# ReplayCoding/mt-renderer

Hardware: AMD Instinct MI355X
Metric: Mtris/sec, 1M-tri 64-bone skinned scene @1920x1080 (higher is better)
Workload: dtype f32; 1 GPU; headline: 20 x mesh50k primitives = 1,000,000 strip triangles, 506,520 vertices x 24 B, 64-bone palette, debug-id shader, 1920x1080; triangles_per_frame=1000000, collective=none

## Files before the change

mt_renderer_amd/csrc/k_geom.hip:

```cpp
#include "geom_bins.h"
#include "geom_vertex.h"

#include <algorithm>
#include <type_traits>

namespace mtr {

struct PV {
    int32_t X, Y;
    float z, iw, up, vp;
    uint32_t flags;
};

enum { OC_XN = 1, OC_XP = 2, OC_YN = 4, OC_YP = 8, OC_ZN = 16, OC_ZP = 32 };

__device__ __forceinline__ uint32_t outcode(const VOut& c) {
    uint32_t oc = 0;
    if (c.x < -c.w) oc |= OC_XN;
    if (c.x > c.w) oc |= OC_XP;
    if (c.y < -c.w) oc |= OC_YN;
    if (c.y > c.w) oc |= OC_YP;
    if (c.z < 0.0f) oc |= OC_ZN;
    if (c.z > c.w) oc |= OC_ZP;
    return oc;
// ... 32 lines not shown
    if (cull == 0u ? A2 <= 0 : (A2 == 0 || (cull == 2u && A2 > 0))) return false;
    const bool flip = A2 < 0;
    const PV& b = flip ? c_in : b_in;
    const PV& c = flip ? b_in : c_in;
    int32_t xmin = min(a.X, min(b.X, c.X)), xmax = max(a.X, max(b.X, c.X));
    int32_t ymin = min(a.Y, min(b.Y, c.Y)), ymax = max(a.Y, max(b.Y, c.Y));
    int32_t px0 = (xmin + 127) >> 8, px1 = (xmax - 128) >> 8;
    int32_t py0 = (ymin + 127) >> 8, py1 = (ymax - 128) >> 8;
    px0 = max(px0, 0); py0 = max(py0, 0);
    px1 = min(px1, (int32_t)W - 1); py1 = min(py1, (int32_t)H - 1);
    if (px0 > px1 || py0 > py1) return false;
    if (small) *small = ((xmax - xmin) | (ymax - ymin)) < 512;
    r.h.bx0 = (uint16_t)(px0 >> MTR_BIN_SHIFT); r.h.bx1 = (uint16_t)(px1 >> MTR_BIN_SHIFT);
    r.h.by0 = (uint16_t)(py0 >> MTR_BIN_SHIFT); r.h.by1 = (uint16_t)(py1 >> MTR_BIN_SHIFT);
    r.a.X0 = a.X; r.a.Y0 = a.Y; r.a.X1 = b.X; r.a.Y1 = b.Y; r.a.X2 = c.X; r.a.Y2 = c.Y;
    r.a.z0 = a.z; r.a.z1 = b.z; r.a.z2 = c.z; r.a.mat = mat; r.a.pad0 = 0; r.a.pad1 = 0;
    r.b.iw0 = a.iw; r.b.iw1 = b.iw; r.b.iw2 = c.iw;
    r.b.up0 = a.up; r.b.up1 = b.up; r.b.up2 = c.up;
    r.b.vp0 = a.vp; r.b.vp1 = b.vp; r.b.vp2 = c.vp;
    r.b.pad0 = r.b.pad1 = r.b.pad2 = 0.0f;
    return true;
}

#ifndef MTR_SAMPLE_CULL
#define MTR_SAMPLE_CULL 1
#endif
#ifndef MTR_SAMPLE_FRAC
#define MTR_SAMPLE_FRAC 2u
#endif
__device__ __forceinline__ bool sample_cull(Rec& r, uint32_t W, uint32_t H) {
    const int32_t xmin = min(r.a.X0, min(r.a.X1, r.a.X2)), xmax = max(r.a.X0, max(r.a.X1, r.a.X2));
    const int32_t ymin = min(r.a.Y0, min(r.a.Y1, r.a.Y2)), ymax = max(r.a.Y0, max(r.a.Y1, r.a.Y2));
    const int32_t px0 = max((xmin + 127) >> 8, 0), py0 = max((ymin + 127) >> 8, 0);
    const bool two_x = min((xmax - 128) >> 8, (int32_t)W - 1) > px0, two_y = min((ymax - 128) >> 8, (int32_t)H - 1) > py0;
    const int32_t Sx = px0 * 256 + 128, Sy = py0 * 256 + 128;
    const int32_t u[3] = {Sx - r.a.X0, Sx - r.a.X1, Sx - r.a.X2}, v[3] = {Sy - r.a.Y0, Sy - r.a.Y1, Sy - r.a.Y2};
    int32_t e[3], ex[3], ey[3];
#pragma unroll
    for (int i = 0; i < 3; i++) {
        const int ia = (i + 1) % 3, ib = (i + 2) % 3;
        const int32_t ndx = u[ib] - u[ia], dy = v[ia] - v[ib];
        const int32_t bias = (((dy << 12) + ndx) - 1) >> 31;
        e[i] = __mul24(u[ib], v[ia]) - __mul24(u[ia], v[ib]) + bias;
        ex[i] = dy << 8; ey[i] = ndx << 8;
    }
    const bool m00 = (e[0] | e[1] | e[2]) >= 0;
    bool m10 = false, m01 = false, m11 = false;
    if (__ballot(two_x || two_y)) {
        m10 = two_x && ((e[0] + ex[0]) | (e[1] + ex[1]) | (e[2] + ex[2])) >= 0;
        m01 = two_y && ((e[0] + ey[0]) | (e[1] + ey[1]) | (e[2] + ey[2])) >= 0;
        m11 = two_x && two_y && ((e[0] + ex[0] + ey[0]) | (e[1] + ex[1] + ey[1]) | (e[2] + ex[2] + ey[2])) >= 0;
    }
    if (!(m00 || m10 || m01 || m11)) return false;
    if (two_x || two_y) {
        const int32_t qx0 = (m00 || m01) ? px0 : px0 + 1, qx1 = (m10 || m11) ? px0 + 1 : px0;
        const int32_t qy0 = (m00 || m10) ? py0 : py0 + 1, qy1 = (m01 || m11) ? py0 + 1 : py0;
        r.h.bx0 = (uint16_t)(qx0 >> MTR_BIN_SHIFT); r.h.bx1 = (uint16_t)(qx1 >> MTR_BIN_SHIFT);
        r.h.by0 = (uint16_t)(qy0 >> MTR_BIN_SHIFT); r.h.by1 = (uint16_t)(qy1 >> MTR_BIN_SHIFT);
    }
    return true;
}

#define MTR_MAX_POLY 8
__device__ __forceinline__ float guard_dist(const VOut& v, int plane) {
    return plane == 0 ? fmaf(64.0f, v.w, -v.x) : plane == 1 ? fmaf(64.0f, v.w, v.x) : plane == 2 ? fmaf(64.0f, v.w, -v.y) : fmaf(64.0f, v.w, v.y);
}
__device__ __forceinline__ VOut plane_lerp(const VOut& in, const VOut& out, float din, float dout) {
    const float t = din / (din - dout);
    VOut r;
    r.x = fmaf(t, out.x - in.x, in.x);
    r.y = fmaf(t, out.y - in.y, in.y);
    r.z = fmaf(t, out.z - in.z, in.z);
    r.w = fmaf(t, out.w - in.w, in.w);
    r.u = fmaf(t, out.u - in.u, in.u);
    r.v = fmaf(t, out.v - in.v, in.v);
    return r;
}
__device__ __forceinline__ VOut clip_lerp(const VOut& in, const VOut& out) {
    VOut r = plane_lerp(in, out, in.z, out.z);
    r.z = 0.0f;
    return r;
}

__device__ __forceinline__ void stage_palette(const GeomParams& P, uint32_t inst, float* s_pal, float* s_M) {
    if (threadIdx.x < 16) {
        float a = P.vp[threadIdx.x];
        if (P.model_mats) a = vp_model_elem(P.vp, P.model_mats, inst, threadIdx.x);
        s_M[threadIdx.x] = a;
    }
    if (P.palettes && P.npal) {
        const float4* src = reinterpret_cast<const float4*>(P.palettes + (size_t)inst * P.pal_stride);
        for (uint32_t i = threadIdx.x; i < P.npal * 4; i += blockDim.x) reinterpret_cast<float4*>(s_pal)[i] = src[i];
    }
    __syncthreads();
}

__device__ __forceinline__ uint32_t shading_position(const DPrim& pr, uint32_t lane) {
    return pr.topology == 4 ? (((lane & 31u) << 1) | (lane >> 5)) : lane;
}
__device__ __forceinline__ uint32_t fetch_index(const GeomParams& P, const DChunk& ch, const DPrim& pr, uint32_t lane) {
    const int32_t ps = (int32_t)ch.start - 2 + (int32_t)shading_position(pr, lane);
    return (ps >= 0 && (uint32_t)ps < pr.index_num) ? (uint32_t)P.ibuf[pr.index_ofs + (uint32_t)ps] : 0xFFFFu;
}

template <int MODE>
__device__ __forceinline__ void geom_chunk(const GeomParams& P, uint32_t inst, uint32_t c, const DChunk& ch, const DPrim& pr,
                                           bool skinned, const float* s_M, const float* s_pal, RecHdr* s_hdr, uint32_t* s_slot,
                                           float4* s_pv, uint32_t lane, uint32_t idx) {
    const uint32_t gid = P.chunk_base + inst * P.nchunks + c;
    const uint32_t mat = P.mat_base + inst * P.mat_inst_stride + ch.prim;
    const uint32_t W = P.fb.W, H = P.fb.H;
    const bool strip = pr.topology == 4;
    const DMat dmat = P.mats[mat];
    const bool want_b = pr.has_uv && dmat.shader == MTR_SH_TEXTURED;

    const uint32_t sp = shading_position(pr, lane);
    {
        const int32_t ps = (int32_t)ch.start - 2 + (int32_t)sp;
        const bool in_s = ps >= 0 && (uint32_t)ps < pr.index_num;
        const bool restart_s = !in_s || (strip && idx == 0xFFFFu);
        const uint32_t vid_s = idx + pr.index_base;
        const bool valid_s = !restart_s && vid_s < pr.vertex_num;
#ifndef MTR_ABL
#define MTR_ABL 0
#endif
#if MTR_ABL == 2
        VOut v; v.x = (float)(vid_s & 1023u) * 0.001f - 0.5f; v.y = (float)(vid_s >> 10) * 0.01f - 0.3f; v.z = 0.5f; v.w = 1.0f; v.u = v.v = 0.0f;
#else
        const VOut v = shade_vertex_mfma(P.vbuf, pr, vid_s, valid_s, s_M, s_pal, P.npal, MTR_ABL == 1 ? false : skinned, want_b);
#endif
        PV q;
        q.X = 0; q.Y = 0; q.z = 0.0f; q.iw = 0.0f; q.up = 0.0f; q.vp = 0.0f; q.flags = 0;
        if (valid_s) {
#if MTR_ABL == 6
            q.X = (int32_t)(v.x * 1000.0f); q.Y = (int32_t)(v.y * 1000.0f); q.z = v.z; q.flags = 2u;
#else
            q = project(v, W, H);
#endif
            q.flags |= 1u | (outcode(v) << 2);
        }
        const uint32_t fw = q.flags | (restart_s ? 0x100u : 0u) | (vid_s << 16);
        s_pv[sp] = make_float4(__int_as_float(q.X), __int_as_float(q.Y), q.z, __uint_as_float(fw));
        if (want_b) s_pv[64 + sp] = make_float4(q.iw, q.up, q.vp, 0.0f);
    }
    __builtin_amdgcn_fence(__ATOMIC_RELEASE, "wavefront");
    __builtin_amdgcn_wave_barrier();
    __builtin_amdgcn_fence(__ATOMIC_ACQUIRE, "wavefront");
    const int32_t p = (int32_t)ch.start - 2 + (int32_t)lane;
    const bool in_range = p >= 0 && (uint32_t)p < pr.index_num;
    PV me;
    me.iw = 0.0f; me.up = 0.0f; me.vp = 0.0f;
    uint32_t vid;
    bool is_restart;
    {
        const float4 a = s_pv[lane];
        const uint32_t fw = __float_as_uint(a.w);
        me.X = __float_as_int(a.x); me.Y = __float_as_int(a.y); me.z = a.z; me.flags = fw & 0xFFu;
        is_restart = (fw & 0x100u) != 0;
        vid = fw >> 16;
        if (want_b) {
            const float4 b = s_pv[64 + lane];
            me.iw = b.x; me.up = b.y; me.vp = b.z;
        }
    }

#if MTR_ABL == 3
    if (me.X == 0x7fffffff) P.fb.counters[CTR_OVERFLOW] = vid;
    return;
#endif
    const uint64_t R = __ballot(is_restart);
    const uint64_t below = R & ((1ull << lane) - 1ull);
    uint32_t q = 0;
    if (!is_restart) q = below ? lane - (63u - (uint32_t)__clzll((long long)below)) : ch.q_before + lane + 1u;
    bool tri, odd;
    if (strip) {
        tri = q >= 3 && lane >= 2;
        odd = ((q - 3) & 1) != 0;
    } else {
        tri = lane >= 2 && in_range && ((uint32_t)p % 3u == 2u);
        odd = false;
    }

    PV v1, v2;
    v1.iw = v1.up = v1.vp = v2.iw = v2.up = v2.vp = 0.0f;
#define MTR_SHR1(x) __builtin_amdgcn_update_dpp((int)(x), (int)(x), 0x138, 0xf, 0xf, false)
    v1.X = MTR_SHR1(me.X); v2.X = MTR_SHR1(v1.X);
    v1.Y = MTR_SHR1(me.Y); v2.Y = MTR_SHR1(v1.Y);
    v1.z = __int_as_float(MTR_SHR1(__float_as_int(me.z))); v2.z = __int_as_float(MTR_SHR1(__float_as_int(v1.z)));
    if (want_b) {
        v1.iw = __int_as_float(MTR_SHR1(__float_as_int(me.iw))); v2.iw = __int_as_float(MTR_SHR1(__float_as_int(v1.iw)));
        v1.up = __int_as_float(MTR_SHR1(__float_as_int(me.up))); v2.up = __int_as_float(MTR_SHR1(__float_as_int(v1.up)));
        v1.vp = __int_as_float(MTR_SHR1(__float_as_int(me.vp))); v2.vp = __int_as_float(MTR_SHR1(__float_as_int(v1.vp)));
    }
    v1.flags = (uint32_t)MTR_SHR1(me.flags); v2.flags = (uint32_t)MTR_SHR1(v1.flags);
    const uint32_t vid1 = (uint32_t)MTR_SHR1(vid), vid2 = (uint32_t)MTR_SHR1(vid1);
#undef MTR_SHR1

    const PV& ta = v2;
    const PV& tb = odd ? me : v1;
    const PV& tc = odd ? v1 : me;

    Rec r0, r1;
    uint32_t n_out = 0;
    bool empty = false;
    bool small = false;
    VOut poly[MTR_MAX_POLY];
    uint32_t n_poly = 0;
    const uint32_t f_and = ta.flags & tb.flags & tc.flags, f_or = ta.flags | tb.flags | tc.flags;
    tri = tri && (f_and & 1u);
    tri = tri && ((f_and >> 2) == 0);
#if MTR_ABL == 5
    tri = tri && ta.X == 0x7ffffff0;
#endif
    if (tri) {
        if (!((f_or >> 2) & OC_ZN) && (f_and & 2u)) {
            if (setup_tri(ta, tb, tc, W, H, mat, pr.cull, r0, &small)) n_out = 1;
        } else {
            const uint32_t ia = vid2, ib = odd ? vid : vid1, ic = odd ? vid1 : vid;
            float M[16];
#pragma unroll
            for (int i = 0; i < 16; i++) M[i] = s_M[i];
            VOut cv[3];
#pragma nounroll
            for (int i = 0; i < 3; i++) cv[i] = shade_vertex(P.vbuf, pr, i == 0 ? ia : (i == 1 ? ib : ic), M, s_pal, P.npal, skinned);
            int n = 3;
            if ((f_or >> 2) & OC_ZN) {
                n = 0;
#pragma unroll
                for (int i = 0; i < 3; i++) {
                    const VOut& pp = cv[i];
                    const VOut& qq = cv[(i + 1) % 3];
                    bool pin = !(pp.z < 0.0f), qin = !(qq.z < 0.0f);
                    if (pin) poly[n++] = pp;
                    if (pin != qin) poly[n++] = pin ? clip_lerp(pp, qq) : clip_lerp(qq, pp);
                }
            } else {
                poly[0] = cv[0]; poly[1] = cv[1]; poly[2] = cv[2];
            }
            if (n >= 3) {
                bool all_ok = true;
                for (int i = 0; i < n; i++) all_ok = all_ok && (project(poly[i], W, H).flags & 2u);
                if (all_ok) {
                    PV q0 = project(poly[0], W, H), q1 = project(poly[1], W, H), q2 = project(poly[2], W, H);
                    bool s0 = setup_tri(q0, q1, q2, W, H, mat, pr.cull, r0);
                    bool s1 = false;
                    if (n == 4) {
                        PV q3 = project(poly[3], W, H);
                        s1 = setup_tri(q0, q2, q3, W, H, mat, pr.cull, s0 ? r1 : r0);
                    }
                    n_out = (s0 ? 1u : 0u) + (s1 ? 1u : 0u);
                } else {
                    VOut tmp[MTR_MAX_POLY];
                    for (int plane = 0; plane < 4 && n >= 3; plane++) {
                        int m = 0;
                        for (int i = 0; i < n; i++) {
                            const VOut pp = poly[i], qq = poly[(i + 1) % n];
                            const float dp = guard_dist(pp, plane), dq = guard_dist(qq, plane);
                            const bool pin = !(dp < 0.0f), qin = !(dq < 0.0f);
                            if (pin && m < MTR_MAX_POLY) tmp[m++] = pp;
                            if (pin != qin && m < MTR_MAX_POLY) tmp[m++] = pin ? plane_lerp(pp, qq, dp, dq) : plane_lerp(qq, pp, dq, dp);
                        }
                        for (int i = 0; i < m; i++) poly[i] = tmp[i];
                        n = m;
                    }
                    if (n >= 3) n_poly = (uint32_t)n;
                }
            }
        }
    }

#if MTR_SAMPLE_CULL
    {
        const uint64_t sm = __ballot(small);
        if (sm && (uint32_t)__popcll(sm) * MTR_SAMPLE_FRAC >= (uint32_t)__popcll(__ballot(n_out != 0u)) && small && !sample_cull(r0, W, H)) {
            n_out = 0;
            empty = true;
        }
    }
#endif
    if (P.fb.own.world > 1 && empty) empty = rect_owned_any(P.fb.own, r0.h.bx0, r0.h.by0, r0.h.bx1, r0.h.by1, P.fb.nbx);
    if (P.fb.own.world > 1 && n_out) {
        const bool k0 = rect_owned_any(P.fb.own, r0.h.bx0, r0.h.by0, r0.h.bx1, r0.h.by1, P.fb.nbx);
        const bool k1 = n_out == 2 && rect_owned_any(P.fb.own, r1.h.bx0, r1.h.by0, r1.h.bx1, r1.h.by1, P.fb.nbx);
        if (!k0 && k1) r0 = r1;
        n_out = (k0 ? 1u : 0u) + (k1 ? 1u : 0u);
    }

    const uint32_t n_res = n_poly ? n_poly - 2u : n_out;
    uint32_t rank, total;
    const uint64_t b1 = __ballot(n_out >= 1), b2 = __ballot(n_out == 2);
    const uint32_t n_empty = (uint32_t)__popcll(__ballot(empty));
    if (!__ballot(n_poly != 0)) {
        const uint64_t lt = (1ull << lane) - 1ull;
        rank = (uint32_t)__popcll(b1 & lt) + (uint32_t)__popcll(b2 & lt);
        total = (uint32_t)__popcll(b1) + (uint32_t)__popcll(b2);
    } else {
        const uint32_t inc = wave_incl_scan_u32(n_res);
        rank = inc - n_res;
        total = (uint32_t)__builtin_amdgcn_readlane((int)inc, 63);
        if (total > MTR_CHUNK_SLOTS) {
            if (lane == 0) atomicOr(&P.fb.counters[CTR_OVERFLOW], 1u);
            total = 0;
        }
    }
    const uint32_t base = gid * MTR_CHUNK_SLOTS;
    if (lane == 0) {
        if (MODE == 0) {
            ChunkInfo ci = {base, total};
            P.fb.chunk_info[gid] = ci;
        }
        const uint32_t nrec = (uint32_t)__popcll(b1) + (uint32_t)__popcll(b2);
        const uint32_t nset = (total ? nrec : 0u) + n_empty;
        if (nset) atomicAdd(&P.fb.counters[MTR_CTR(CTR_REC, gid)], nset);
    }
    total = __builtin_amdgcn_readfirstlane(total);
    if (total == 0) return;
    const uint32_t solid = (dmat.shader != MTR_SH_TEXTURED && dmat.blend != MTR_DB_ADD && dmat.dstate == 3u) ? 1u : 0u;
    const uint32_t hard = (dmat.blend == MTR_DB_ADD || dmat.dstate != 3u) ? 1u : 0u;
    const uint32_t mflags = solid | ((dmat.blend != MTR_DB_OFF ? 1u : 0u) << 8) | (dmat.translucent << 16) | (hard << 17);
    r0.a.pad0 = dmat.rgba8; r0.a.pad1 = mflags;
    r1.a.pad0 = dmat.rgba8; r1.a.pad1 = mflags;
    auto put_rec = [&](uint32_t slot, const Rec& r) {
        const bool lg = rec_is_large(r.a);
        P.fb.rec_a[base + slot] = rec_pack(r.a, lg);
        if (lg) P.fb.rec_l[base + slot] = make_int4(r.a.X1, r.a.Y1, r.a.X2, r.a.Y2);
        if (MODE == 0) P.fb.rec_hdr[base + slot] = r.h;
        if (want_b) P.fb.rec_b[base + slot] = r.b;
        s_hdr[slot] = r.h;
    };
    if (n_out >= 1) put_rec(rank, r0);
    if (n_out == 2) put_rec(rank + 1, r1);
    if (n_poly) {
        uint32_t nvalid = 0;
        for (uint32_t k = 0; k + 2u < n_poly; k++) {
            Rec t;
            const PV q0 = project(poly[0], W, H), q1 = project(poly[k + 1], W, H), q2 = project(poly[k + 2], W, H);
            bool ok = setup_tri(q0, q1, q2, W, H, mat, pr.cull, t);
            if (ok && P.fb.own.world > 1) ok = rect_owned_any(P.fb.own, t.h.bx0, t.h.by0, t.h.bx1, t.h.by1, P.fb.nbx);
            if (ok) {
                t.a.pad0 = dmat.rgba8; t.a.pad1 = mflags;
                put_rec(rank + k, t);
                nvalid++;
            } else {
                const RecHdr hole = {1, 1, 0, 0};
                s_hdr[rank + k] = hole;
                if (MODE == 0) P.fb.rec_hdr[base + rank + k] = hole;
            }
        }
        if (nvalid) atomicAdd(&P.fb.counters[MTR_CTR(CTR_REC, gid + lane)], nvalid);
    }
    __builtin_amdgcn_fence(__ATOMIC_RELEASE, "wavefront");
    __builtin_amdgcn_wave_barrier();
    __builtin_amdgcn_fence(__ATOMIC_ACQUIRE, "wavefront");

#if MTR_ABL == 4
    return;
#endif
    for (uint32_t round = 0; round * 64 < total; ++round) {
        const uint32_t j = round * 64 + lane;
        bool act = j < total;
        RecHdr h = {0, 0, 0, 0};
        if (act) h = s_hdr[j];
        act = act && h.bx0 <= h.bx1;
        if (MODE == 2) {
            emit_bins_unordered(P.fb, h, act, gid, round, lane, s_slot);
        } else if (MODE == 1) {
            emit_bins<true>(P.fb, h, act, gid, round, lane);
        } else {
            count_bins(P.fb, h, act, lane);
        }
    }
}

#ifndef GEOM_OCC
#define GEOM_OCC 8
#define GEOM_OCC_SMALL 7
#endif
template <int MODE, bool CULL, int OCC>
__global__ __launch_bounds__(256, OCC) void k_geom(GeomParams P) {
    extern __shared__ __align__(16) float s_pal[];
    __shared__ RecHdr s_hdr[4][MTR_CHUNK_SLOTS + 4];
    __shared__ uint32_t s_slot[MODE == 2 ? 4 : 1][128];
    __shared__ float4 s_pv[4][128];
    __shared__ float s_M[16];
    const uint32_t lane = threadIdx.x & 63;
    const uint32_t wave = __builtin_amdgcn_readfirstlane(threadIdx.x >> 6);
    if (!CULL) {
        const uint32_t nblk = gridDim.x;
        const uint32_t per = (nblk + 7) / 8;
        const uint32_t blk = (blockIdx.x & 7) * per + (blockIdx.x >> 3);
        const uint32_t c = blk * 4 + wave;
        if (blk >= nblk) return;
        const bool has = c < P.nchunks;
        DChunk ch = {};
        DPrim pr = {};
        uint32_t idx = 0xFFFFu;
        if (has) { ch = P.chunks[c]; pr = P.prims[ch.prim]; idx = fetch_index(P, ch, pr, lane); }
        stage_palette(P, blockIdx.y, s_pal, s_M);
        if (!has) return;
        geom_chunk<MODE>(P, blockIdx.y, c, ch, pr, pr.skinnable && P.palettes && P.npal, s_M, s_pal, s_hdr[wave], s_slot[wave], s_pv[wave], lane, idx);
        return;
    }
    const uint32_t nxq = P.work_nx * 4u, ii = blockIdx.x / nxq, xq = blockIdx.x - ii * nxq, x = xq >> 2, q = xq & 3u;
    const uint32_t nlive = live_instances(P.inst_count, P.ninst);
    if (ii >= nlive) return;
    const size_t mi = (size_t)ii * P.work_nx + x;
    const uint32_t mword = reinterpret_cast<const uint32_t*>(P.work_mask)[mi >> 1];
    const uint32_t inst = P.inst_list ? P.inst_list[ii] : ii;
    const uint32_t m16 = (mi & 1u) ? mword >> 16 : mword & 0xFFFFu;
    const uint32_t k = (uint32_t)__popc(m16);
    if (q * 4u >= k) return;
    const uint32_t nth = q * 4u + wave;
    const bool has = nth < k;
    uint32_t mm = m16;
    for (uint32_t t = 0; t < nth && mm; t++) mm &= mm - 1u;
    const uint32_t c = x * 16u + (mm ? (uint32_t)__ffs((int)mm) - 1u : 0u);
    DChunk ch = {};
    DPrim pr = {};
    uint32_t idx = 0xFFFFu;
    if (has) { ch = P.chunks[c]; pr = P.prims[ch.prim]; idx = fetch_index(P, ch, pr, lane); }
    stage_palette(P, inst, s_pal, s_M);
    if (!has) return;
    geom_chunk<MODE>(P, inst, c, ch, pr, pr.skinnable && P.palettes && P.npal, s_M, s_pal, s_hdr[wave], s_slot[wave], s_pv[wave], lane, idx);
}

#define MTR_GEOM_REST_SPLIT 16u
template <int MODE>
__global__ __launch_bounds__(256) void k_geom_rest(GeomParams P) {
    extern __shared__ __align__(16) float s_pal[];
    __shared__ RecHdr s_hdr[4][MTR_CHUNK_SLOTS + 4];
    __shared__ uint32_t s_slot[MODE == 2 ? 4 : 1][128];
    __shared__ float4 s_pv[4][128];
    __shared__ float s_M[16];
    const uint32_t lane = threadIdx.x & 63;
    const uint32_t wave = __builtin_amdgcn_readfirstlane(threadIdx.x >> 6);
    const uint32_t split = min(P.work_nx, P.rest_split);
    const uint32_t ii = P.work_slot_base + blockIdx.x / split;
    const uint32_t nlive = live_instances(P.inst_count, P.ninst);
    if (ii >= nlive) return;
    const uint32_t inst = P.inst_list ? P.inst_list[ii] : ii;
    stage_palette(P, inst, s_pal, s_M);
    for (uint32_t x = blockIdx.x % split; x < P.work_nx; x += split) {
        const uint32_t m16 = P.work_mask[(size_t)ii * P.work_nx + x];
        const uint32_t k = (uint32_t)__popc(m16);
        for (uint32_t nth = wave; nth < k; nth += 4) {
            uint32_t mm = m16;
            for (uint32_t t = 0; t < nth; t++) mm &= mm - 1u;
            const uint32_t c = x * 16u + (uint32_t)__ffs((int)mm) - 1u;
            const DChunk ch = P.chunks[c];
            const DPrim pr = P.prims[ch.prim];
            geom_chunk<MODE>(P, inst, c, ch, pr, pr.skinnable && P.palettes && P.npal, s_M, s_pal, s_hdr[wave], s_slot[wave], s_pv[wave], lane,
                             fetch_index(P, ch, pr, lane));
        }
    }
}
__global__ __launch_bounds__(256) void k_vertex_stage(GeomParams P, uint32_t prim, float* out_clip, float* out_uv) {
    extern __shared__ __align__(16) float s_pal[];
    __shared__ float s_M[16];
    stage_palette(P, 0, s_pal, s_M);
    const DPrim pr = P.prims[prim];
    const bool skinned = pr.skinnable && P.palettes && P.npal;
    const uint32_t v = blockIdx.x * blockDim.x + threadIdx.x;
    if ((v & ~63u) >= pr.vertex_num) return;
    const VOut o = shade_vertex_mfma(P.vbuf, pr, v, v < pr.vertex_num, s_M, s_pal, P.npal, skinned, true);
    if (v >= pr.vertex_num) return;
    out_clip[4 * v + 0] = o.x; out_clip[4 * v + 1] = o.y; out_clip[4 * v + 2] = o.z; out_clip[4 * v + 3] = o.w;
    out_uv[2 * v + 0] = o.u; out_uv[2 * v + 1] = o.v;
}

}

template <class F>
static void with_geom_mode(const FrameBuffers& fb, F launch) {
    if (fb.direct && fb.unordered) launch(std::integral_constant<int, 2>());
    else if (fb.direct) launch(std::integral_constant<int, 1>());
    else launch(std::integral_constant<int, 0>());
}
template <bool CULL>
static void launch_geom(const GeomParams& p, dim3 grid, size_t lds, hipStream_t s) {
    with_geom_mode(p.fb, [&](auto mode) {
        constexpr int MODE = decltype(mode)::value;
        if (p.small_draw) hipLaunchKernelGGL((mtr::k_geom<MODE, CULL, GEOM_OCC_SMALL>), grid, dim3(256), lds, s, p);
        else hipLaunchKernelGGL((mtr::k_geom<MODE, CULL, GEOM_OCC>), grid, dim3(256), lds, s, p);
    });
}
void mtr_launch_geom(const GeomParams& p, hipStream_t s) {
    if (p.nchunks == 0 || p.ninst == 0) return;
    size_t lds = (size_t)p.npal * 64;
    if (p.work_mask) {
        uint32_t slots = p.ninst;
        if (p.inst_count && p.fb.own.world > 1) slots = std::min<uint32_t>(p.ninst, (2u * p.ninst + p.fb.own.world - 1) / p.fb.own.world + 64u);
        if (p.inst_count && (p.slots_hint & 0x80000000u)) {
            const uint32_t h = p.slots_hint & 0x7FFFFFFFu;
            slots = std::min<uint32_t>(p.ninst, h + h / 8u + 4u);
        }
        if ((uint64_t)(p.ninst - slots) * p.work_nx * 4u <= 20000u) slots = p.ninst;
        if (p.slots_override) slots = std::min<uint32_t>(p.ninst, p.slots_override);
        dim3 grid(p.work_nx * 4u * slots);
        launch_geom<true>(p, grid, lds, s);
        if (slots < p.ninst) {
            GeomParams r = p;
            r.work_slot_base = slots;
            r.rest_split = (p.inst_count && (p.slots_hint & 0x80000000u) && !p.slots_override) ? MTR_GEOM_REST_SPLIT / 4u : MTR_GEOM_REST_SPLIT;
            dim3 rest((p.ninst - slots) * std::min<uint32_t>(p.work_nx, r.rest_split));
            with_geom_mode(p.fb, [&](auto mode) { hipLaunchKernelGGL((mtr::k_geom_rest<decltype(mode)::value>), rest, dim3(256), lds, s, r); });
        }
        return;
    }
    uint32_t nblk = (p.nchunks + 3) / 4;
    nblk = (nblk + 7) / 8 * 8;
    dim3 grid(nblk, p.ninst);
    launch_geom<false>(p, grid, lds, s);
}

void mtr_launch_vertex_stage(const GeomParams& p, uint32_t prim, float* out_clip, float* out_uv, hipStream_t s) {
    hipLaunchKernelGGL(mtr::k_vertex_stage, dim3(256), dim3(256), (size_t)p.npal * 64, s, p, prim, out_clip, out_uv);
}
```

mt_renderer_amd/csrc/mtr_internal.h:

```cpp
#pragma once
#include <hip/hip_runtime.h>
#include <stdint.h>

#define MTR_BIN 16
#define MTR_BIN_SHIFT 4
#define MTR_SUB 8
#define MTR_CHUNK_NEW 62
#define MTR_CHUNK_SLOTS 124
#define MTR_GUARD_BAND 1048576.0f

enum { MTR_SH_DEBUG = 0, MTR_SH_TEXTURED = 1, MTR_SH_CONST = 2 };

struct DPrim {
    uint32_t vertex_base, vertex_num, stride;
    uint32_t index_ofs, index_num, index_base;
    uint32_t topology;
    uint32_t pos_fmt, pos_cnt, pos_off;
    uint32_t uv_fmt, uv_cnt, uv_off, has_uv;
    uint32_t joint_off, weight_off, skinnable;
    uint32_t aligned4;
    uint32_t parts_no;
    uint32_t cull;
};

struct DChunk {
    uint32_t prim;
    uint32_t start;
    uint32_t q_before;
    uint32_t ntris;
    uint32_t b_first;
    uint32_t b_count;
    uint32_t b_flags;
    uint32_t pad;
};

struct BoneBox {
    float cx, cy, cz;
    float ex, ey, ez;
    uint32_t joint;
    uint32_t pad;
};
#define MTR_BOX_UNSKINNED 0xFFFFFFFFu
#define MTR_CULL_CTR_WORDS 32
#define MTR_CHUNK_MAX_BOXES 15

struct CompMat {
    float C[12];
    float A[12];
};

struct DMat {
    uint32_t shader;
    uint32_t rgba8;
    uint32_t blend;
    uint32_t tw, th;
    uint32_t translucent;
    const uint8_t* tex;
    uint32_t tlevels;
    uint32_t dstate;
};
enum { MTR_TR_RGBA8 = 0, MTR_TR_BC1 = 1, MTR_TR_BC7 = 2 };
enum { MTR_DB_OFF = 0, MTR_DB_ALPHA = 1, MTR_DB_ADD = 2 };

struct RecHdr {
    uint16_t bx0, by0, bx1, by1;
};
struct RecA {
    int32_t X0, Y0, X1, Y1;
    int32_t X2, Y2;
    float z0, z1;
    float z2;
    uint32_t mat;
    uint32_t pad0, pad1;
};
struct RecP {
    uint4 q0, q1;
};
#define MTR_REC_LARGE_SENTINEL 0x8000u
#define MTR_MAX_TEXTURED_MATERIALS (1u << 24)

__device__ __forceinline__ bool rec_is_large(const RecA& a) {
    const int32_t d1x = a.X1 - a.X0, d1y = a.Y1 - a.Y0, d2x = a.X2 - a.X0, d2y = a.Y2 - a.Y0;
    return d1x < -32767 || d1x > 32767 || d1y < -32767 || d1y > 32767 || d2x < -32767 || d2x > 32767 || d2y < -32767 || d2y > 32767;
}
// ... 93 lines not shown

template <int CTRL, class T>
__device__ __forceinline__ T dpp_mov(T v) {
    return __builtin_bit_cast(T, __builtin_amdgcn_update_dpp(0, __builtin_bit_cast(int, v), CTRL, 0xf, 0xf, false));
}
template <class T, class Op>
__device__ __forceinline__ T row_reduce(T v, Op op) {
    v = op(v, dpp_mov<0x128>(v));
    v = op(v, dpp_mov<0x124>(v));
    v = op(v, dpp_mov<0x122>(v));
    v = op(v, dpp_mov<0x121>(v));
    return v;
}
template <class T, class Op>
__device__ __forceinline__ T wave_reduce(T v, Op op) {
    v = row_reduce(v, op);
    const int i = __builtin_bit_cast(int, v);
    const T r0 = __builtin_bit_cast(T, __builtin_amdgcn_readlane(i, 0)), r1 = __builtin_bit_cast(T, __builtin_amdgcn_readlane(i, 16));
    const T r2 = __builtin_bit_cast(T, __builtin_amdgcn_readlane(i, 32)), r3 = __builtin_bit_cast(T, __builtin_amdgcn_readlane(i, 48));
    return op(op(r0, r1), op(r2, r3));
}

__device__ __forceinline__ float vp_model_elem(const float (&vp)[16], const float* model_mats, uint32_t inst, uint32_t e) {
    __builtin_assume(e < 16);
    const uint32_t i = e & 3u, c = e >> 2;
    const float* B = model_mats + (size_t)inst * 16;
    float a = 0.0f;
#pragma unroll
    for (int k = 0; k < 4; k++) a = fmaf(vp[k * 4 + i], B[c * 4 + k], a);
    return a;
}

__device__ __forceinline__ uint32_t live_instances(const uint32_t* count, uint32_t ninst) {
    asm("" : "+s"(ninst));
    if (count) ninst = *count;
    return ninst;
}
#endif

enum { CTR_ENTRIES = 1, CTR_SEGS = 2, CTR_OVERFLOW = 3, CTR_SHARD_BASE = 32, CTR_SHARD_STRIDE = 32, CTR_NSHARDS = 128,
       CTR_REC = 0, CTR_ENT = 1, CTR_SEG = 2, CTR_CULL = 3 ,
       CTR_NUM = CTR_SHARD_BASE + CTR_NSHARDS * CTR_SHARD_STRIDE };
#define MTR_CTR(kind, k) (CTR_SHARD_BASE + ((k) & (CTR_NSHARDS - 1)) * CTR_SHARD_STRIDE + (kind))

struct FrameBuffers {
    RecHdr* rec_hdr;
    RecP* rec_a;
    int4* rec_l;
    RecB* rec_b;
    ChunkInfo* chunk_info;
    unsigned long long* bin_count;
    unsigned long long* bin_fill;
    uint32_t* bin_start;
    uint32_t* seg_start;
    uint32_t* entries;
    Seg* segs;
    uint32_t* counters;
    uint32_t rec_cap, entry_cap, seg_cap;
    uint32_t W, H, nbx, nby;
    Ownership own;
    uint32_t direct, qcap, scap;
    uint32_t unordered;
};

__device__ __forceinline__ void bin_queue_done(const FrameBuffers& fb, uint32_t bin) {
    if (fb.direct) {
        fb.bin_count[bin] = fb.bin_fill[bin];
        fb.bin_fill[bin] = 0ull;
    }
}

__device__ __forceinline__ void bin_queue(const FrameBuffers& fb, uint32_t bin, uint32_t& ent_lo, uint32_t& n_ent,
                                          uint32_t& seg_lo, uint32_t& n_seg) {
    if (fb.direct) {
        const unsigned long long f = fb.bin_fill[bin];
        ent_lo = bin * fb.qcap; seg_lo = bin * fb.scap;
        n_ent = min((uint32_t)f, fb.qcap); n_seg = min((uint32_t)(f >> 32), fb.scap);
    } else {
        ent_lo = fb.bin_start[bin]; n_ent = fb.bin_start[bin + 1] - ent_lo;
        seg_lo = fb.seg_start[bin]; n_seg = fb.seg_start[bin + 1] - seg_lo;
    }
}

struct GeomParams {
    const uint8_t* vbuf;
    const uint16_t* ibuf;
    const DPrim* prims;
    const DChunk* chunks;
    const BoneBox* boxes;
    uint32_t nchunks;
    uint32_t ninst;
    const uint16_t* work_mask;
    uint32_t work_nx;
    uint32_t work_slot_base;
    uint32_t rest_split;
    uint32_t slots_override;
    uint32_t small_draw;
    const uint32_t* inst_list;
    const uint32_t* inst_count;
    uint32_t slots_hint;
    const float* model_mats;
    const float* palettes;
    uint32_t npal, pal_stride;
    float vp[16];
    uint32_t chunk_base;
    uint32_t mat_base, mat_inst_stride;
    const DMat* mats;
    FrameBuffers fb;
};

struct alignas(64) TileHead {
    uint32_t grid;
    uint32_t own_count;
    uint32_t nbx, nbins;
    uint32_t W, H;
    uint32_t direct, qcap, scap;
    uint32_t xcd_run;
    uint32_t nbx_mul, nbx_shift, run_mul, run_shift;
    uint32_t zero_nwords, nhint;
    const uint32_t* own_list;
    uint32_t* entries;
    unsigned long long* bin_fill;
    uint32_t* bin_start;
    uint32_t* seg_start;
    uint32_t* counters;
    RecP* rec_a;
    uint32_t* zero_next;
    uint32_t* zero_words;
    uint32_t* host_status;
};
static_assert(sizeof(TileHead) == 192 && alignof(TileHead) == 64, "TileHead is three 64-byte lines");

struct TileParams {
    TileHead head;
    FrameBuffers fb;
    const DMat* mats;
    uint8_t* color;
    float* depth;
    uint32_t clear_rgba8;
    float clear_depth;
    uint8_t* bin_flag;
    uint32_t mixed;
    uint32_t* zero_next;
    uint32_t* host_status;
    uint32_t vis_waves;
    uint32_t xcd_run;
    uint32_t* zero_words;
    uint32_t zero_nwords;
    uint32_t* hint_out;
    uint32_t nhint;
    uint16_t hint_word[4], hint_slot[4];
};
#define MTR_TILE_PARAMS 1

static inline uint32_t mtr_vis_waves_for(uint32_t forced, uint32_t own_count) {
    if (forced) return forced;
    return own_count <= 1536 ? 8u : own_count <= 4096 ? 4u : 2u;
}

void mtr_launch_geom(const GeomParams& p, hipStream_t s);
void mtr_launch_scan(const FrameBuffers& fb, hipStream_t s);
void mtr_launch_fill(const FrameBuffers& fb, uint32_t total_chunks, hipStream_t s);
void mtr_launch_tile(const TileParams& p, bool textured, hipStream_t s);
void mtr_launch_tile_vis(const TileParams& p, bool textured, hipStream_t s);
void mtr_launch_alpha_min(const uint8_t* rgba, size_t npixels, uint32_t* out_min, hipStream_t s);
void mtr_launch_vertex_stage(const GeomParams& p, uint32_t prim, float* out_clip, float* out_uv, hipStream_t s);
void mtr_launch_bc1_decode(const uint8_t* blocks, uint8_t* rgba, uint32_t w, uint32_t h, hipStream_t s);
void mtr_launch_bc7_decode(const uint8_t* blocks, uint8_t* rgba, uint32_t w, uint32_t h, hipStream_t s);
void mtr_launch_pack_shard(const uint8_t* color, uint8_t* dst, uint32_t W, uint32_t H, const uint32_t* own_list, uint32_t own_count,
                           uint32_t stride_bins, hipStream_t s);
void mtr_launch_unpack_shards(const uint8_t* gathered, uint8_t* color, uint32_t W, uint32_t H, const uint32_t* src_of_bin, hipStream_t s);
struct CullParams {
    const BoneBox* boxes;
    uint32_t nboxes;
    uint32_t ninst;
    const float* model_mats;
    const float* palettes;
    uint32_t npal, pal_stride;
    float vp[16];
    uint32_t W, H, nbx, nby;
    Ownership own;
    uint32_t* list;
    uint32_t* count;
    CompMat* comp;
    uint32_t ncomp;
    uint16_t* work_mask;
    uint32_t* strad;
    uint32_t nchunks;
    uint32_t* counters;
};
void mtr_launch_cull_instances(const CullParams& p, hipStream_t s);
struct ChunkCullParams {
// ... 163 lines not shown
```

Before: 23430 Mtris/s.

## Pack hot geometry kernel args into cache-line head and overlap palette loads

Adds a 256-byte, 64-byte-aligned GeomHead at the start of the kernel arguments holding the hot scalars, pointers and VP matrix, read through scalar loads. Cold framebuffer fields are reloaded late from the kernarg segment. Palette staging is split into an issue phase and a finish phase so the palette global loads overlap the chunk, prim and material fetches. Material rows can also be prefetched alongside prims for the small-occupancy variant. This aims to cut kernel-prologue latency and scalar-load stalls, at the cost of a larger kernarg block and fragile inline-asm scheduling hints.

```diff
diff --git a/mt_renderer_amd/csrc/k_geom.hip b/mt_renderer_amd/csrc/k_geom.hip
--- a/mt_renderer_amd/csrc/k_geom.hip
+++ b/mt_renderer_amd/csrc/k_geom.hip
@@ -138,36 +138,128 @@
     return r;
 }
 
-__device__ __forceinline__ void stage_palette(const GeomParams& P, uint32_t inst, float* s_pal, float* s_M) {
-    if (threadIdx.x < 16) {
-        float a = P.vp[threadIdx.x];
-        if (P.model_mats) a = vp_model_elem(P.vp, P.model_mats, inst, threadIdx.x);
+#define MTR_GEOM_BLOCK 256u
+struct PalStage {
+    float4 v0;
+    float a[4], b[4];
+    const float4* src;
+    uint32_t n4;
+    bool composed;
+};
+__device__ __forceinline__ PalStage palette_issue(const GeomParams& P, const GeomHead& h, uint32_t inst, float* s_M) {
+    PalStage st;
+    st.v0 = make_float4(0.0f, 0.0f, 0.0f, 0.0f);
+#pragma unroll
+    for (int k = 0; k < 4; k++) st.a[k] = st.b[k] = 0.0f;
+    st.n4 = h.palettes ? h.npal * 4 : 0u;
+    st.src = reinterpret_cast<const float4*>(h.palettes + (size_t)inst * h.pal_stride);
+    st.composed = h.model_mats != nullptr;
+    if (threadIdx.x < st.n4) st.v0 = st.src[threadIdx.x];
+    if (st.composed) {
+        if (threadIdx.x < 16) {
+            const uint32_t i = threadIdx.x & 3u, c = threadIdx.x >> 2;
+            const float* B = h.model_mats + (size_t)inst * 16;
+#pragma unroll
+            for (int k = 0; k < 4; k++) { st.a[k] = P.vp[k * 4 + i]; st.b[k] = B[c * 4 + k]; }
+        }
+    } else if (threadIdx.x == 0) {
+#pragma unroll
+        for (int c = 0; c < 4; c++) reinterpret_cast<float4*>(s_M)[c] = make_float4(h.vp[c * 4], h.vp[c * 4 + 1], h.vp[c * 4 + 2], h.vp[c * 4 + 3]);
+    }
+    return st;
+}
+__device__ __forceinline__ void palette_finish(const PalStage& st, float* s_pal, float* s_M) {
+    if (st.composed && threadIdx.x < 16) {
+        float a = 0.0f;
+        PalStage t = st;
+        asm volatile("" : "+v"(t.a[0]), "+v"(t.a[1]), "+v"(t.a[2]), "+v"(t.a[3]), "+v"(t.b[0]), "+v"(t.b[1]), "+v"(t.b[2]), "+v"(t.b[3]));
+#pragma unroll
+        for (int k = 0; k < 4; k++) a = fmaf(t.a[k], t.b[k], a);
         s_M[threadIdx.x] = a;
     }
-    if (P.palettes && P.npal) {
-        const float4* src = reinterpret_cast<const float4*>(P.palettes + (size_t)inst * P.pal_stride);
-        for (uint32_t i = threadIdx.x; i < P.npal * 4; i += blockDim.x) reinterpret_cast<float4*>(s_pal)[i] = src[i];
-    }
+    if (threadIdx.x < st.n4) reinterpret_cast<float4*>(s_pal)[threadIdx.x] = st.v0;
+    for (uint32_t i = threadIdx.x + MTR_GEOM_BLOCK; i < st.n4; i += MTR_GEOM_BLOCK) reinterpret_cast<float4*>(s_pal)[i] = st.src[i];
     __syncthreads();
+}
+__device__ __forceinline__ void stage_palette(const GeomParams& P, const GeomHead& h, uint32_t inst, float* s_pal, float* s_M) {
+    const PalStage st = palette_issue(P, h, inst, s_M);
+    palette_finish(st, s_pal, s_M);
+}
+
+template <bool CULL>
+__device__ __forceinline__ GeomHead geom_head(const GeomParams& P) {
+    const GeomHead h = P.head;
+    asm volatile("" ::"s"(h.grid), "s"(h.nchunks), "s"(h.chunk_base), "s"(h.mat_base), "s"(h.mat_inst_stride), "s"(h.npal), "s"(h.pal_stride),
+                 "s"(h.chunks), "s"(h.prims), "s"(h.ibuf), "s"(h.vbuf), "s"(h.mats), "s"(h.palettes), "s"(h.model_mats), "s"(h.W), "s"(h.H),
+                 "s"(h.world));
+    asm volatile("" ::"s"(h.vp[0]), "s"(h.vp[1]), "s"(h.vp[2]), "s"(h.vp[3]), "s"(h.vp[4]), "s"(h.vp[5]), "s"(h.vp[6]), "s"(h.vp[7]), "s"(h.vp[8]),
+                 "s"(h.vp[9]), "s"(h.vp[10]), "s"(h.vp[11]), "s"(h.vp[12]), "s"(h.vp[13]), "s"(h.vp[14]), "s"(h.vp[15]));
+    if (CULL) asm volatile("" ::"s"(h.ninst), "s"(h.work_nx), "s"(h.work_mask), "s"(h.inst_list), "s"(h.inst_count));
+    return h;
+}
+typedef const __attribute__((address_space(4))) uint32_t* ConstWords;
+template <class T>
+__device__ __forceinline__ T load_words(ConstWords q) {
+    static_assert(sizeof(T) % 4 == 0 && alignof(T) >= 4, "whole dwords");
+    struct Words { uint32_t w[sizeof(T) / 4]; } r;
+#pragma unroll
+    for (uint32_t i = 0; i < sizeof(T) / 4; i++) r.w[i] = q[i];
+    return __builtin_bit_cast(T, r);
+}
+template <class T>
+__device__ __forceinline__ T load_const(const T* p) {
+    return load_words<T>((ConstWords)p);
+}
+
+__device__ __forceinline__ FrameBuffers geom_late(const GeomHead& h) {
+    typedef const GeomParams __attribute__((address_space(4)))* GeomArgs;
+    GeomArgs q = (GeomArgs)__builtin_amdgcn_kernarg_segment_ptr();
+    asm volatile("" : "+s"(q));
+    FrameBuffers fb = load_words<FrameBuffers>((ConstWords)&q->fb);
+    fb.rec_a = q->head.rec_a; fb.rec_l = q->head.rec_l; fb.rec_b = q->head.rec_b;
+    fb.entries = q->head.entries; fb.bin_fill = q->head.bin_fill; fb.counters = q->head.counters;
+    fb.nbx = q->head.nbx; fb.qcap = q->head.qcap;
+    asm volatile("" ::"s"(fb.rec_a), "s"(fb.rec_l), "s"(fb.rec_b), "s"(fb.entries), "s"(fb.bin_fill), "s"(fb.counters), "s"(fb.nbx), "s"(fb.qcap));
+    fb.W = h.W; fb.H = h.H;
+    fb.own.world = h.world;
+    return fb;
+}
+
+__device__ __forceinline__ uint32_t geom_live_instances(const GeomHead& h) {
+    uint32_t n = h.ninst;
+    asm("" : "+s"(n));
+    if (h.inst_count) n = load_const(h.inst_count);
+    return n;
 }
 
 __device__ __forceinline__ uint32_t shading_position(const DPrim& pr, uint32_t lane) {
     return pr.topology == 4 ? (((lane & 31u) << 1) | (lane >> 5)) : lane;
 }
-__device__ __forceinline__ uint32_t fetch_index(const GeomParams& P, const DChunk& ch, const DPrim& pr, uint32_t lane) {
+__device__ __forceinline__ uint32_t fetch_index(const GeomHead& h, const DChunk& ch, const DPrim& pr, uint32_t lane) {
     const int32_t ps = (int32_t)ch.start - 2 + (int32_t)shading_position(pr, lane);
-    return (ps >= 0 && (uint32_t)ps < pr.index_num) ? (uint32_t)P.ibuf[pr.index_ofs + (uint32_t)ps] : 0xFFFFu;
-}
-
-template <int MODE>
-__device__ __forceinline__ void geom_chunk(const GeomParams& P, uint32_t inst, uint32_t c, const DChunk& ch, const DPrim& pr,
-                                           bool skinned, const float* s_M, const float* s_pal, RecHdr* s_hdr, uint32_t* s_slot,
+    return (ps >= 0 && (uint32_t)ps < pr.index_num) ? (uint32_t)h.ibuf[pr.index_ofs + (uint32_t)ps] : 0xFFFFu;
+}
+template <bool ROW>
+__device__ __forceinline__ void fetch_prim_mat(const GeomHead& h, uint32_t inst, const DChunk& ch, DPrim& pr, DMat& dm) {
+    pr = load_const(h.prims + ch.prim);
+    if (ROW) {
+        dm = load_const(h.mats + (h.mat_base + inst * h.mat_inst_stride + ch.prim));
+        asm volatile("" ::"s"(pr.index_ofs), "s"(dm.shader), "s"(dm.rgba8), "s"(dm.blend), "s"(dm.translucent), "s"(dm.dstate));
+    } else {
+        asm volatile("" ::"s"(pr.index_ofs));
+    }
+    __builtin_amdgcn_sched_barrier(0);
+}
+
+template <int MODE, bool ROW>
+__device__ __forceinline__ void geom_chunk(const GeomHead& P, uint32_t inst, uint32_t c, const DChunk& ch,
+                                           const DPrim& pr, const DMat& row, bool skinned, const float* s_M, const float* s_pal, RecHdr* s_hdr, uint32_t* s_slot,
                                            float4* s_pv, uint32_t lane, uint32_t idx) {
     const uint32_t gid = P.chunk_base + inst * P.nchunks + c;
     const uint32_t mat = P.mat_base + inst * P.mat_inst_stride + ch.prim;
-    const uint32_t W = P.fb.W, H = P.fb.H;
+    const uint32_t W = P.W, H = P.H;
     const bool strip = pr.topology == 4;
-    const DMat dmat = P.mats[mat];
+    const DMat dmat = ROW ? row : load_const(P.mats + mat);
     const bool want_b = pr.has_uv && dmat.shader == MTR_SH_TEXTURED;
 
     const uint32_t sp = shading_position(pr, lane);
@@ -221,7 +313,7 @@
     }
 
 #if MTR_ABL == 3
-    if (me.X == 0x7fffffff) P.fb.counters[CTR_OVERFLOW] = vid;
+    if (me.X == 0x7fffffff) P.counters[CTR_OVERFLOW] = vid;
     return;
 #endif
     const uint64_t R = __ballot(is_restart);
@@ -325,6 +417,7 @@
         }
     }
 
+    const FrameBuffers fb = geom_late(P);
 #if MTR_SAMPLE_CULL
     {
         const uint64_t sm = __ballot(small);
@@ -334,10 +427,10 @@
         }
     }
 #endif
-    if (P.fb.own.world > 1 && empty) empty = rect_owned_any(P.fb.own, r0.h.bx0, r0.h.by0, r0.h.bx1, r0.h.by1, P.fb.nbx);
-    if (P.fb.own.world > 1 && n_out) {
-        const bool k0 = rect_owned_any(P.fb.own, r0.h.bx0, r0.h.by0, r0.h.bx1, r0.h.by1, P.fb.nbx);
-        const bool k1 = n_out == 2 && rect_owned_any(P.fb.own, r1.h.bx0, r1.h.by0, r1.h.bx1, r1.h.by1, P.fb.nbx);
+    if (P.world > 1 && empty) empty = rect_owned_any(fb.own, r0.h.bx0, r0.h.by0, r0.h.bx1, r0.h.by1, fb.nbx);
+    if (P.world > 1 && n_out) {
+        const bool k0 = rect_owned_any(fb.own, r0.h.bx0, r0.h.by0, r0.h.bx1, r0.h.by1, fb.nbx);
+        const bool k1 = n_out == 2 && rect_owned_any(fb.own, r1.h.bx0, r1.h.by0, r1.h.bx1, r1.h.by1, fb.nbx);
         if (!k0 && k1) r0 = r1;
         n_out = (k0 ? 1u : 0u) + (k1 ? 1u : 0u);
     }
@@ -355,7 +448,7 @@
         rank = inc - n_res;
         total = (uint32_t)__builtin_amdgcn_readlane((int)inc, 63);
         if (total > MTR_CHUNK_SLOTS) {
-            if (lane == 0) atomicOr(&P.fb.counters[CTR_OVERFLOW], 1u);
+            if (lane == 0) atomicOr(&fb.counters[CTR_OVERFLOW], 1u);
             total = 0;
         }
     }
@@ -363,11 +456,11 @@
     if (lane == 0) {
         if (MODE == 0) {
             ChunkInfo ci = {base, total};
-            P.fb.chunk_info[gid] = ci;
+            fb.chunk_info[gid] = ci;
         }
         const uint32_t nrec = (uint32_t)__popcll(b1) + (uint32_t)__popcll(b2);
         const uint32_t nset = (total ? nrec : 0u) + n_empty;
-        if (nset) atomicAdd(&P.fb.counters[MTR_CTR(CTR_REC, gid)], nset);
+        if (nset) atomicAdd(&fb.counters[MTR_CTR(CTR_REC, gid)], nset);
     }
     total = __builtin_amdgcn_readfirstlane(total);
     if (total == 0) return;
@@ -378,10 +471,10 @@
     r1.a.pad0 = dmat.rgba8; r1.a.pad1 = mflags;
     auto put_rec = [&](uint32_t slot, const Rec& r) {
         const bool lg = rec_is_large(r.a);
-        P.fb.rec_a[base + slot] = rec_pack(r.a, lg);
-        if (lg) P.fb.rec_l[base + slot] = make_int4(r.a.X1, r.a.Y1, r.a.X2, r.a.Y2);
-        if (MODE == 0) P.fb.rec_hdr[base + slot] = r.h;
-        if (want_b) P.fb.rec_b[base + slot] = r.b;
+        fb.rec_a[base + slot] = rec_pack(r.a, lg);
+        if (lg) fb.rec_l[base + slot] = make_int4(r.a.X1, r.a.Y1, r.a.X2, r.a.Y2);
+        if (MODE == 0) fb.rec_hdr[base + slot] = r.h;
+        if (want_b) fb.rec_b[base + slot] = r.b;
         s_hdr[slot] = r.h;
     };
     if (n_out >= 1) put_rec(rank, r0);
@@ -392,7 +485,7 @@
             Rec t;
             const PV q0 = project(poly[0], W, H), q1 = project(poly[k + 1], W, H), q2 = project(poly[k + 2], W, H);
             bool ok = setup_tri(q0, q1, q2, W, H, mat, pr.cull, t);
-            if (ok && P.fb.own.world > 1) ok = rect_owned_any(P.fb.own, t.h.bx0, t.h.by0, t.h.bx1, t.h.by1, P.fb.nbx);
+            if (ok && P.world > 1) ok = rect_owned_any(fb.own, t.h.bx0, t.h.by0, t.h.bx1, t.h.by1, fb.nbx);
             if (ok) {
                 t.a.pad0 = dmat.rgba8; t.a.pad1 = mflags;
                 put_rec(rank + k, t);
@@ -400,10 +493,10 @@
             } else {
                 const RecHdr hole = {1, 1, 0, 0};
                 s_hdr[rank + k] = hole;
-                if (MODE == 0) P.fb.rec_hdr[base + rank + k] = hole;
+                if (MODE == 0) fb.rec_hdr[base + rank + k] = hole;
             }
         }
-        if (nvalid) atomicAdd(&P.fb.counters[MTR_CTR(CTR_REC, gid + lane)], nvalid);
+        if (nvalid) atomicAdd(&fb.counters[MTR_CTR(CTR_REC, gid + lane)], nvalid);
     }
     __builtin_amdgcn_fence(__ATOMIC_RELEASE, "wavefront");
     __builtin_amdgcn_wave_barrier();
@@ -419,11 +512,11 @@
         if (act) h = s_hdr[j];
         act = act && h.bx0 <= h.bx1;
         if (MODE == 2) {
-            emit_bins_unordered(P.fb, h, act, gid, round, lane, s_slot);
+            emit_bins_unordered(fb, h, act, gid, round, lane, s_slot);
         } else if (MODE == 1) {
-            emit_bins<true>(P.fb, h, act, gid, round, lane);
+            emit_bins<true>(fb, h, act, gid, round, lane);
         } else {
-            count_bins(P.fb, h, act, lane);
+            count_bins(fb, h, act, lane);
         }
     }
 }
@@ -438,34 +531,39 @@
     __shared__ RecHdr s_hdr[4][MTR_CHUNK_SLOTS + 4];
     __shared__ uint32_t s_slot[MODE == 2 ? 4 : 1][128];
     __shared__ float4 s_pv[4][128];
-    __shared__ float s_M[16];
+    __shared__ __align__(16) float s_M[16];
     const uint32_t lane = threadIdx.x & 63;
     const uint32_t wave = __builtin_amdgcn_readfirstlane(threadIdx.x >> 6);
+    constexpr bool ROW = OCC == GEOM_OCC_SMALL;
+    const GeomHead h = geom_head<CULL>(P);
     if (!CULL) {
-        const uint32_t nblk = gridDim.x;
+        const uint32_t nblk = h.grid;
         const uint32_t per = (nblk + 7) / 8;
         const uint32_t blk = (blockIdx.x & 7) * per + (blockIdx.x >> 3);
         const uint32_t c = blk * 4 + wave;
         if (blk >= nblk) return;
-        const bool has = c < P.nchunks;
+        const PalStage st = palette_issue(P, h, blockIdx.y, s_M);
+        const bool has = c < h.nchunks;
         DChunk ch = {};
         DPrim pr = {};
+        DMat dm = {};
         uint32_t idx = 0xFFFFu;
-        if (has) { ch = P.chunks[c]; pr = P.prims[ch.prim]; idx = fetch_index(P, ch, pr, lane); }
-        stage_palette(P, blockIdx.y, s_pal, s_M);
+        if (has) { ch = load_const(h.chunks + c); fetch_prim_mat<ROW>(h, blockIdx.y, ch, pr, dm); idx = fetch_index(h, ch, pr, lane); }
+        palette_finish(st, s_pal, s_M);
         if (!has) return;
-        geom_chunk<MODE>(P, blockIdx.y, c, ch, pr, pr.skinnable && P.palettes && P.npal, s_M, s_pal, s_hdr[wave], s_slot[wave], s_pv[wave], lane, idx);
+        geom_chunk<MODE, ROW>(h, blockIdx.y, c, ch, pr, dm, pr.skinnable && st.n4, s_M, s_pal, s_hdr[wave], s_slot[wave], s_pv[wave], lane, idx);
         return;
     }
-    const uint32_t nxq = P.work_nx * 4u, ii = blockIdx.x / nxq, xq = blockIdx.x - ii * nxq, x = xq >> 2, q = xq & 3u;
-    const uint32_t nlive = live_instances(P.inst_count, P.ninst);
+    const uint32_t nxq = h.work_nx * 4u, ii = blockIdx.x / nxq, xq = blockIdx.x - ii * nxq, x = xq >> 2, q = xq & 3u;
+    const uint32_t nlive = geom_live_instances(h);
     if (ii >= nlive) return;
-    const size_t mi = (size_t)ii * P.work_nx + x;
-    const uint32_t mword = reinterpret_cast<const uint32_t*>(P.work_mask)[mi >> 1];
-    const uint32_t inst = P.inst_list ? P.inst_list[ii] : ii;
+    const size_t mi = (size_t)ii * h.work_nx + x;
+    const uint32_t mword = load_const(reinterpret_cast<const uint32_t*>(h.work_mask) + (mi >> 1));
+    const uint32_t inst = h.inst_list ? load_const(h.inst_list + ii) : ii;
     const uint32_t m16 = (mi & 1u) ? mword >> 16 : mword & 0xFFFFu;
     const uint32_t k = (uint32_t)__popc(m16);
     if (q * 4u >= k) return;
+    const PalStage st = palette_issue(P, h, inst, s_M);
     const uint32_t nth = q * 4u + wave;
     const bool has = nth < k;
     uint32_t mm = m16;
@@ -473,11 +571,12 @@
     const uint32_t c = x * 16u + (mm ? (uint32_t)__ffs((int)mm) - 1u : 0u);
     DChunk ch = {};
     DPrim pr = {};
+    DMat dm = {};
     uint32_t idx = 0xFFFFu;
-    if (has) { ch = P.chunks[c]; pr = P.prims[ch.prim]; idx = fetch_index(P, ch, pr, lane); }
-    stage_palette(P, inst, s_pal, s_M);
+    if (has) { ch = load_const(h.chunks + c); fetch_prim_mat<ROW>(h, inst, ch, pr, dm); idx = fetch_index(h, ch, pr, lane); }
+    palette_finish(st, s_pal, s_M);
     if (!has) return;
-    geom_chunk<MODE>(P, inst, c, ch, pr, pr.skinnable && P.palettes && P.npal, s_M, s_pal, s_hdr[wave], s_slot[wave], s_pv[wave], lane, idx);
+    geom_chunk<MODE, ROW>(h, inst, c, ch, pr, dm, pr.skinnable && st.n4, s_M, s_pal, s_hdr[wave], s_slot[wave], s_pv[wave], lane, idx);
 }
 
 #define MTR_GEOM_REST_SPLIT 16u
@@ -487,38 +586,42 @@
     __shared__ RecHdr s_hdr[4][MTR_CHUNK_SLOTS + 4];
     __shared__ uint32_t s_slot[MODE == 2 ? 4 : 1][128];
     __shared__ float4 s_pv[4][128];
-    __shared__ float s_M[16];
+    __shared__ __align__(16) float s_M[16];
     const uint32_t lane = threadIdx.x & 63;
     const uint32_t wave = __builtin_amdgcn_readfirstlane(threadIdx.x >> 6);
-    const uint32_t split = min(P.work_nx, P.rest_split);
+    const GeomHead h = geom_head<true>(P);
+    const uint32_t split = min(h.work_nx, P.rest_split);
     const uint32_t ii = P.work_slot_base + blockIdx.x / split;
-    const uint32_t nlive = live_instances(P.inst_count, P.ninst);
+    const uint32_t nlive = geom_live_instances(h);
     if (ii >= nlive) return;
-    const uint32_t inst = P.inst_list ? P.inst_list[ii] : ii;
-    stage_palette(P, inst, s_pal, s_M);
-    for (uint32_t x = blockIdx.x % split; x < P.work_nx; x += split) {
-        const uint32_t m16 = P.work_mask[(size_t)ii * P.work_nx + x];
+    const uint32_t inst = h.inst_list ? load_const(h.inst_list + ii) : ii;
+    stage_palette(P, h, inst, s_pal, s_M);
+    for (uint32_t x = blockIdx.x % split; x < h.work_nx; x += split) {
+        const uint32_t m16 = h.work_mask[(size_t)ii * h.work_nx + x];
         const uint32_t k = (uint32_t)__popc(m16);
         for (uint32_t nth = wave; nth < k; nth += 4) {
             uint32_t mm = m16;
             for (uint32_t t = 0; t < nth; t++) mm &= mm - 1u;
             const uint32_t c = x * 16u + (uint32_t)__ffs((int)mm) - 1u;
-            const DChunk ch = P.chunks[c];
-            const DPrim pr = P.prims[ch.prim];
-            geom_chunk<MODE>(P, inst, c, ch, pr, pr.skinnable && P.palettes && P.npal, s_M, s_pal, s_hdr[wave], s_slot[wave], s_pv[wave], lane,
-                             fetch_index(P, ch, pr, lane));
+            const DChunk ch = load_const(h.chunks + c);
+            DPrim pr;
+            DMat dm;
+            fetch_prim_mat<true>(h, inst, ch, pr, dm);
+            geom_chunk<MODE, true>(h, inst, c, ch, pr, dm, pr.skinnable && h.palettes && h.npal, s_M, s_pal, s_hdr[wave], s_slot[wave], s_pv[wave], lane,
+                             fetch_index(h, ch, pr, lane));
         }
     }
 }
 __global__ __launch_bounds__(256) void k_vertex_stage(GeomParams P, uint32_t prim, float* out_clip, float* out_uv) {
     extern __shared__ __align__(16) float s_pal[];
-    __shared__ float s_M[16];
-    stage_palette(P, 0, s_pal, s_M);
-    const DPrim pr = P.prims[prim];
-    const bool skinned = pr.skinnable && P.palettes && P.npal;
-    const uint32_t v = blockIdx.x * blockDim.x + threadIdx.x;
+    __shared__ __align__(16) float s_M[16];
+    const GeomHead h = geom_head<false>(P);
+    stage_palette(P, h, 0, s_pal, s_M);
+    const DPrim pr = load_const(h.prims + prim);
+    const bool skinned = pr.skinnable && h.palettes && h.npal;
+    const uint32_t v = blockIdx.x * MTR_GEOM_BLOCK + threadIdx.x;
     if ((v & ~63u) >= pr.vertex_num) return;
-    const VOut o = shade_vertex_mfma(P.vbuf, pr, v, v < pr.vertex_num, s_M, s_pal, P.npal, skinned, true);
+    const VOut o = shade_vertex_mfma(h.vbuf, pr, v, v < pr.vertex_num, s_M, s_pal, h.npal, skinned, true);
     if (v >= pr.vertex_num) return;
     out_clip[4 * v + 0] = o.x; out_clip[4 * v + 1] = o.y; out_clip[4 * v + 2] = o.z; out_clip[4 * v + 3] = o.w;
     out_uv[2 * v + 0] = o.u; out_uv[2 * v + 1] = o.v;
@@ -540,8 +643,10 @@
         else hipLaunchKernelGGL((mtr::k_geom<MODE, CULL, GEOM_OCC>), grid, dim3(256), lds, s, p);
     });
 }
-void mtr_launch_geom(const GeomParams& p, hipStream_t s) {
-    if (p.nchunks == 0 || p.ninst == 0) return;
+void mtr_launch_geom(const GeomParams& params, hipStream_t s) {
+    if (params.nchunks == 0 || params.ninst == 0) return;
+    GeomParams p = params;
+    geom_fill_head(p);
     size_t lds = (size_t)p.npal * 64;
     if (p.work_mask) {
         uint32_t slots = p.ninst;
@@ -563,12 +668,12 @@
         }
         return;
     }
-    uint32_t nblk = (p.nchunks + 3) / 4;
-    nblk = (nblk + 7) / 8 * 8;
-    dim3 grid(nblk, p.ninst);
+    dim3 grid(p.head.grid, p.ninst);
     launch_geom<false>(p, grid, lds, s);
 }
 
-void mtr_launch_vertex_stage(const GeomParams& p, uint32_t prim, float* out_clip, float* out_uv, hipStream_t s) {
+void mtr_launch_vertex_stage(const GeomParams& params, uint32_t prim, float* out_clip, float* out_uv, hipStream_t s) {
+    GeomParams p = params;
+    geom_fill_head(p);
     hipLaunchKernelGGL(mtr::k_vertex_stage, dim3(256), dim3(256), (size_t)p.npal * 64, s, p, prim, out_clip, out_uv);
 }
diff --git a/mt_renderer_amd/csrc/mtr_internal.h b/mt_renderer_amd/csrc/mtr_internal.h
--- a/mt_renderer_amd/csrc/mtr_internal.h
+++ b/mt_renderer_amd/csrc/mtr_internal.h
@@ -1,5 +1,6 @@
 #pragma once
 #include <hip/hip_runtime.h>
+#include <stddef.h>
 #include <stdint.h>
 
 #define MTR_BIN 16
@@ -259,7 +260,40 @@
     }
 }
 
+struct alignas(64) GeomHead {
+    uint32_t grid;
+    uint32_t nchunks, ninst;
+    uint32_t chunk_base, mat_base, mat_inst_stride;
+    uint32_t npal, pal_stride;
+    const DChunk* chunks;
+    const DPrim* prims;
+    const uint16_t* ibuf;
+    const uint8_t* vbuf;
+    const DMat* mats;
+    const float* palettes;
+    const float* model_mats;
+    uint32_t W, H;
+    uint32_t world;
+    uint32_t work_nx;
+    const uint16_t* work_mask;
+    const uint32_t* inst_list;
+    const uint32_t* inst_count;
+    RecP* rec_a;
+    int4* rec_l;
+    RecB* rec_b;
+    uint32_t* entries;
+    unsigned long long* bin_fill;
+    uint32_t* counters;
+    uint32_t nbx;
+    uint32_t qcap, direct;
+    uint32_t pad;
+    float vp[16];
+};
+static_assert(sizeof(GeomHead) == 256 && alignof(GeomHead) == 64, "GeomHead is four 64-byte lines");
+static_assert(offsetof(GeomHead, mats) == 64 && offsetof(GeomHead, rec_a) == 128 && offsetof(GeomHead, vp) == 192, "one line each");
+
 struct GeomParams {
+    GeomHead head;
     const uint8_t* vbuf;
     const uint16_t* ibuf;
     const DPrim* prims;
@@ -285,6 +319,24 @@
     const DMat* mats;
     FrameBuffers fb;
 };
+inline void geom_fill_head(GeomParams& p) {
+    GeomHead& h = p.head;
+    h.grid = ((p.nchunks + 3) / 4 + 7) / 8 * 8;
+    h.nchunks = p.nchunks; h.ninst = p.ninst;
+    h.chunk_base = p.chunk_base; h.mat_base = p.mat_base; h.mat_inst_stride = p.mat_inst_stride;
+    h.npal = p.npal; h.pal_stride = p.pal_stride;
+    h.chunks = p.chunks; h.prims = p.prims; h.ibuf = p.ibuf; h.vbuf = p.vbuf;
+    h.mats = p.mats; h.palettes = p.palettes; h.model_mats = p.model_mats;
+    h.W = p.fb.W; h.H = p.fb.H; h.nbx = p.fb.nbx;
+    h.world = p.fb.own.world;
+    h.direct = p.fb.direct; h.qcap = p.fb.qcap;
+    h.work_nx = p.work_nx;
+    h.pad = 0;
+    h.rec_a = p.fb.rec_a; h.rec_l = p.fb.rec_l; h.rec_b = p.fb.rec_b;
+    h.entries = p.fb.entries; h.bin_fill = p.fb.bin_fill; h.counters = p.fb.counters;
+    h.work_mask = p.work_mask; h.inst_list = p.inst_list; h.inst_count = p.inst_count;
+    for (int i = 0; i < 16; i++) h.vp[i] = p.vp[i];
+}
 
 struct alignas(64) TileHead {
     uint32_t grid;
```

Result: no change. 23850 Mtris/s (median of 6 runs) (+1.8%).
